# astro-turing/Integrating-diagenetic-equations-using-Python

Hardware: AMD Instinct MI355X
Metric: grid-point-steps/sec (5 fields, fp64) (higher is better)
Workload: dtype f64

## Files before the change

integrating-diagenetic-equations-using-python_amd/csrc/marl_kernels.h:

```cpp
#pragma once
#include <type_traits>

#include "marl_math.h"
#include "marl_brent.h"

namespace marl {

enum : int { LAYOUT_FIELD_MAJOR = 0, LAYOUT_TILED = 1 };

template <int LAYOUT>
__device__ __forceinline__ int64_t at(int f, int64_t i, int64_t ld)
{
    if constexpr (LAYOUT == LAYOUT_FIELD_MAJOR)
        return (int64_t)f * ld + i;
    else
        return (i >> 6) * (int64_t)(NF * 64) + f * 64 + (i & 63);
}

struct Slab {
    int64_t n_buf;
    int64_t goff;
    int64_t ld;
    int64_t out_lo;
    int64_t out_hi;
};

__device__ __forceinline__ double nanmin(double a, double b) { return (a < b || a != a) ? a : b; }
__device__ __forceinline__ double nanmax(double a, double b) { return (a > b || a != a) ? a : b; }
template <bool FINITE = false>
__device__ __forceinline__ double mon_min(double a, double b) { return FINITE ? __builtin_fmin(a, b) : nanmin(a, b); }
template <bool FINITE = false>
__device__ __forceinline__ double mon_max(double a, double b) { return FINITE ? __builtin_fmax(a, b) : nanmax(a, b); }


#ifdef MARL_LAB_PHASE_CLOCK
__device__ unsigned long long marl_lab_phase[8];
#define MARL_PHASE_MARK(k) do { const unsigned long long t_ = __builtin_amdgcn_s_memtime(); ph_acc[k] += t_ - ph_last; ph_last = t_; } while (0)
#else
#define MARL_PHASE_MARK(k) do { } while (0)
#endif

#define MARL_ONCE _Pragma("unroll") for (int once_ = 0; once_ < 1; once_++)
#define MARL_FIELDS _Pragma("unroll") for (int f = 0; f < NF; f++)

template <int BLK, bool REUSE = true, bool VD = false, int SEAM = 0>
struct StencilBlock {
    static constexpr int EDGE_DOUBLES = 2 * NF * BLK;
    static constexpr bool CACHE_LDS = PC_LDS_SLOTS > 0;
    static constexpr bool CACHE = REUSE && (EDGE_DOUBLES + TABLE_DOUBLES + PC_LDS_SLOTS * BLK) * 8 <= 60 * 1024;
    static constexpr int CACHE_DOUBLES = CACHE ? PC_LDS_SLOTS * BLK : 0;
    static constexpr int LDS_DOUBLES = EDGE_DOUBLES + TABLE_DOUBLES + CACHE_DOUBLES;

    double* lds;
    Tables T;
    HotConsts K;
    const DevConsts* C;
    int tid;
    int parity;
    unsigned masks;
    static constexpr bool EDGE_ONCE = CACHE;
    unsigned edge_cells;
    __device__ __forceinline__ bool edge_wave() const
    {
        if constexpr (EDGE_ONCE) return edge_cells & 1u;
        else return __builtin_amdgcn_ballot_w64(is_edge() != 0) != 0;
    }
    __device__ __forceinline__ unsigned is_first() const { return masks & 1u; }
    __device__ __forceinline__ unsigned is_last() const { return (masks >> 8) & 1u; }
    __device__ __forceinline__ unsigned in_zone() const { return (masks >> 16) & 1u; }
    __device__ __forceinline__ unsigned is_edge() const { return masks & 0x101u; }
    PointCache<(CACHE && CACHE_LDS) ? BLK : 0> cache;
    bool reuse_live = false;
    static constexpr int SEAM_STRIDE = 16, SEAM_READS = 0x10000, SEAM_WAVE0 = 0x20000, SEAM_WAVEW = 0x40000;
    static_assert(SEAM < BLK, "the recording lane is a lane of the window");
    double* seam = nullptr;
    int seam_pos = 0;
#ifdef MARL_LAB_PHASE_CLOCK
    unsigned long long ph_acc[6] = {0, 0, 0, 0, 0, 0}, ph_last = __builtin_amdgcn_s_memtime();
    __device__ __forceinline__ void phase_flush()
    {
        if (threadIdx.x == 0)
            for (int k = 0; k < 6; k++) atomicAdd(&marl_lab_phase[k], ph_acc[k]);
    }
#endif

    __device__ __forceinline__ StencilBlock(double* lds_, int64_t g0, const DevConsts* __restrict__ c)
        : lds(lds_), T(load_tables(lds_ + EDGE_DOUBLES, BLK)), K(load_hot(c)), C(c), tid(threadIdx.x), parity(0)
    {
        set_window(g0);
        if constexpr (CACHE && CACHE_LDS) cache.s = lds_ + EDGE_DOUBLES + TABLE_DOUBLES + tid;
    }

    __device__ __forceinline__ void rebind(int t)
    {
        tid = t;
        if constexpr (CACHE && CACHE_LDS) cache.s = lds + EDGE_DOUBLES + TABLE_DOUBLES + t;
    }

    __device__ __forceinline__ void set_window(int64_t g)
    {
        const int64_t N = C->N, mlo = C->mask_lo, mhi = C->mask_hi;
        masks = ((g == 0) ? 1u : 0u) | ((g == N - 1) ? 0x100u : 0u) | ((g >= mlo && g < mhi) ? 0x10000u : 0u);
        edge_cells = 0;
        if constexpr (EDGE_ONCE) edge_cells = (__builtin_amdgcn_ballot_w64(is_edge() != 0) != 0) ? 1u : 0u;
    }

    template <int MODE = TR_PLAIN>
    __device__ __forceinline__ void eval(const double (&ys)[NF], double (&k)[NF], PointAux& aux)
    {
        MARL_PHASE_MARK(4);
        double* e = lds + parity * (NF * BLK);
#pragma unroll
        for (int f = 0; f < NF; f++) e[f * BLK + tid] = ys[f];
        if constexpr (SEAM > 0) {
            if (seam_pos & SEAM_WAVEW) {
                int tw = tid;
                asm volatile("" : "+v"(tw));
                if (tw == SEAM) {
                    double* rec = seam + (seam_pos & 0xffff);
#pragma unroll
                    for (int f = 0; f < NF; f++) rec[f] = ys[f];
                }
            }
        }
        MARL_PHASE_MARK(0);
        PointLocal pl;
        MARL_ONCE point_local<CACHE ? MODE : TR_PLAIN, (CACHE && CACHE_LDS) ? BLK : 0, VD>(ys, in_zone(), K, C, T, pl, aux, cache, reuse_live);
        MARL_PHASE_MARK(1);
        __syncthreads();
        MARL_PHASE_MARK(2);
        const int tl = tid > 0 ? tid - 1 : 0;
        const int tr = tid < BLK - 1 ? tid + 1 : BLK - 1;
        double left[NF], right[NF];
#pragma unroll
        for (int f = 0; f < NF; f++) left[f] = e[f * BLK + tl];
        if constexpr (SEAM > 0) {
            if ((seam_pos & (SEAM_WAVE0 | SEAM_READS)) == (SEAM_WAVE0 | SEAM_READS)) {
                int t0 = tid;
                asm volatile("" : "+v"(t0));
                if (t0 == 0) {
                    const double* prev = seam + ((seam_pos & 0xffff) ^ 8);
#pragma unroll
                    for (int f = 0; f < NF; f++) left[f] = prev[f];
                }
            }
            seam_pos += SEAM_STRIDE;
        }
        const bool need_right_solids = __builtin_amdgcn_ballot_w64(!pl.upw) != 0;
        if constexpr (CACHE) {
#pragma unroll
            for (int f = 2; f < NF; f++) right[f] = e[f * BLK + tr];
            asm volatile("" : "=v"(right[0]), "=v"(right[1]));
            if (need_right_solids) {
                right[0] = e[tr];
                right[1] = e[BLK + tr];
            }
        } else {
#pragma unroll
            for (int f = 0; f < NF; f++) right[f] = (f >= 2 || need_right_solids) ? e[f * BLK + tr] : 0.0;
        }
        parity ^= 1;
        MARL_ONCE {
            double um[NF], up[NF];
#pragma unroll
            for (int f = 0; f < NF; f++) { um[f] = left[f]; up[f] = right[f]; }
            if (edge_wave()) {
                if (is_last()) {
#pragma unroll
                    for (int f = 0; f < NF; f++) up[f] = ghost_upper(f, ys[f], um[f]);
                }
                if (is_first()) {
#pragma unroll
                    for (int f = 0; f < NF; f++) um[f] = ghost_lower(C->bc[f], ys[f]);
                }
            }
            point_rates<VD, true, !CACHE>(ys, um, up, K, T, pl, k, need_right_solids);
        }
#ifdef MARL_LAB_PHASE_CLOCK
        asm volatile("" :: "v"(k[0]), "v"(k[4]));
        MARL_PHASE_MARK(3);
        ph_acc[5]++;
#endif
    }
};

template <int BLK, int NQ, int NMIN, bool FINITE = false>
__device__ __forceinline__ void block_reduce(double (&q)[NQ], double* scratch)
{
    const int lane = threadIdx.x & 63, wave = threadIdx.x >> 6;
    constexpr int NW = BLK / 64;
    auto combine = [](int j, double a, double o) { return (j == 0) ? a + o : (j <= NMIN ? mon_min<FINITE>(a, o) : mon_max<FINITE>(a, o)); };
    if constexpr (NW > 1) {
        __syncthreads();
#pragma unroll
        for (int j = 0; j < NQ; j++) scratch[j * BLK + threadIdx.x] = q[j];
        __syncthreads();
#pragma unroll
        for (int jj = 0; jj < (NQ + NW - 1) / NW; jj++) {
            const int j = wave + jj * NW;
            if (j < NQ) {
                double a = scratch[j * BLK + lane];
#pragma unroll
                for (int i = 1; i < NW; i++) a = combine(j, a, scratch[j * BLK + lane + 64 * i]);
#pragma unroll
                for (int off = 32; off > 0; off >>= 1) a = combine(j, a, __shfl_xor(a, off, 64));
                if (lane == 0) scratch[j * BLK] = a;
            }
        }
        __syncthreads();
        if (threadIdx.x == 0) {
#pragma unroll
            for (int j = 0; j < NQ; j++) q[j] = scratch[j * BLK];
        }
        __syncthreads();
    } else {
#pragma unroll
        for (int off = 32; off > 0; off >>= 1) {
#pragma unroll
            for (int j = 0; j < NQ; j++) q[j] = combine(j, q[j], __shfl_xor(q[j], off, 64));
        }
    }
}

struct ZBatch {
    int64_t zstride;
    const int32_t* act;
    int64_t act_stride;
    int want;
    const int32_t* list;
};
__device__ __forceinline__ int64_t z_inst(const ZBatch& B)
{
    return B.list ? (int64_t)__builtin_amdgcn_readfirstlane(B.list[blockIdx.z]) : (int64_t)blockIdx.z;
}
__device__ __forceinline__ bool z_masked_out(const ZBatch& B)
{
    return B.act && !(*reinterpret_cast<const int32_t*>(reinterpret_cast<const char*>(B.act) + z_inst(B) * B.act_stride) & B.want);
}
template <class P>
__device__ __forceinline__ P* z_shift(P* p, const ZBatch& B)
{
    return reinterpret_cast<P*>(reinterpret_cast<char*>(const_cast<typename std::remove_const<P>::type*>(p)) + z_inst(B) * B.zstride);
}

template <int LAYOUT, bool VD = false>
__global__ void __launch_bounds__(256) rhs_kernel(const double* __restrict__ y, double* __restrict__ dydt,
                                                  const DevConsts* __restrict__ consts, Slab S, int64_t inst_stride, int const_stride,
                                                  ZBatch B = ZBatch{0, nullptr, 0, 0, nullptr})
{
    if (z_masked_out(B)) return;
    __shared__ double tabs[TABLE_DOUBLES];
    const Tables T = load_tables(tabs, 256);
    const DevConsts& C = consts[blockIdx.y * const_stride + z_inst(B)];
    y = z_shift(y, B) + blockIdx.y * inst_stride;
    dydt = z_shift(dydt, B) + blockIdx.y * inst_stride;
    const int64_t l = (int64_t)blockIdx.x * 256 + threadIdx.x;
    if (l < S.out_lo || l >= S.out_hi) return;
    const int64_t g = l + S.goff;
    double uc[NF], um[NF], up[NF], r[NF];
    PointAux aux;
#pragma unroll
    for (int f = 0; f < NF; f++) {
        uc[f] = y[at<LAYOUT>(f, l, S.ld)];
        um[f] = (g > 0) ? y[at<LAYOUT>(f, l - 1, S.ld)] : ghost_lower(C.bc[f], uc[f]);
    }
#pragma unroll
    for (int f = 0; f < NF; f++) up[f] = (g < C.N - 1) ? y[at<LAYOUT>(f, l + 1, S.ld)] : ghost_upper(f, uc[f], um[f]);
    const HotConsts K = load_hot(&C);
    PointCache<0> pc;
    bool live = false;
    rhs_point<TR_PLAIN, 0, VD>(uc, um, up, g >= C.mask_lo && g < C.mask_hi, K, &C, T, r, aux, pc, live);
#pragma unroll
    for (int f = 0; f < NF; f++) dydt[at<LAYOUT>(f, l, S.ld)] = r[f];
}

__global__ void __launch_bounds__(256) math_probe_kernel(int op, const double* __restrict__ x, double* __restrict__ y, int64_t n, double e)
{
    __shared__ double tabs[TABLE_DOUBLES];
    const Tables T = load_tables(tabs, 256);
    const int64_t i = (int64_t)blockIdx.x * 256 + threadIdx.x;
    if (i >= n) return;
    const double v = x[i];
    double r;
    switch (op) {
        case 0: r = fast_log(v, T); break;
        case 1: r = fast_exp(v, T); break;
        case 2: r = pow_sat(v, e, T); break;
        case 3: r = rcp_nr(v); break;
        case 4: r = fv_sigma<false>(v, e, T); break;
        default: r = fv_sigma<true>(v, e, T); break;
    }
    y[i] = r;
}

template <int SRC, int DST>
__global__ void __launch_bounds__(256) convert_kernel(const double* __restrict__ src, double* __restrict__ dst, int64_t n,
                                                      int64_t ld_src, int64_t ld_dst, int64_t stride_src, int64_t stride_dst)
{
    src += blockIdx.y * stride_src;
    dst += blockIdx.y * stride_dst;
    const int64_t i = (int64_t)blockIdx.x * 256 + threadIdx.x;
    if (i >= n) return;
#pragma unroll
    for (int f = 0; f < NF; f++) dst[at<DST>(f, i, ld_dst)] = src[at<SRC>(f, i, ld_src)];
}

constexpr int NQ = 8;
constexpr int NQMIN = 4;

__device__ __forceinline__ void monitors_init(double (&q)[NQ])
{
    q[0] = 0.0;
    q[1] = q[2] = q[3] = q[4] = __builtin_inf();
    q[5] = q[6] = q[7] = -__builtin_inf();
}

template <bool FINITE = false>
__device__ __forceinline__ void monitors_accumulate(double (&q)[NQ], const double (&u)[NF], double U, double W)
{
    q[1] = mon_min<FINITE>(mon_min<FINITE>(mon_min<FINITE>(mon_min<FINITE>(mon_min<FINITE>(q[1], u[0]), u[1]), u[2]), u[3]), u[4]);
    q[2] = mon_min<FINITE>(q[2], u[0]);
    q[3] = mon_min<FINITE>(q[3], u[1]);
    q[4] = mon_min<FINITE>(q[4], U);
    q[5] = mon_max<FINITE>(q[5], u[0] + u[1]);
    q[6] = mon_max<FINITE>(q[6], u[4]);
    q[7] = mon_max<FINITE>(q[7], W);
}

template <int LAYOUT>
__global__ void __launch_bounds__(256) monitors_kernel(const double* __restrict__ y, const DevConsts* __restrict__ consts,
                                                       Slab S, int64_t inst_stride, double* __restrict__ part)
{
    __shared__ double scratch[NQ * 256];
    __shared__ double tabs[TABLE_DOUBLES];
    const Tables T = load_tables(tabs, 256);
    const DevConsts& C = consts[blockIdx.y];
    y += blockIdx.y * inst_stride;
    double q[NQ];
    monitors_init(q);
    for (int64_t l = S.out_lo + (int64_t)blockIdx.x * 256 + threadIdx.x; l < S.out_hi; l += (int64_t)gridDim.x * 256) {
        double u[NF];
#pragma unroll
        for (int f = 0; f < NF; f++) u[f] = y[at<LAYOUT>(f, l, S.ld)];
        const double Phi = u[4];
        const double F = 1.0 - fast_exp(10.0 - 10.0 * rcp_nr(Phi), T);
        const double rF = C.hot.rhorat * F;
        monitors_accumulate(q, u, C.hot.presum + rF * (Phi * Phi * Phi) * rcp_nr(1.0 - Phi), C.hot.presum - rF * Phi * Phi);
    }
    block_reduce<256, NQ, NQMIN>(q, scratch);
    if (threadIdx.x == 0) {
        double* p = part + ((int64_t)blockIdx.y * gridDim.x + blockIdx.x) * NQ;
#pragma unroll
        for (int j = 0; j < NQ; j++) p[j] = q[j];
    }
}

__global__ void __launch_bounds__(256) reduce_records_kernel(const double* __restrict__ part, int64_t nblocks, double* __restrict__ out)
{
    __shared__ double scratch[NQ * 256];
    part += (int64_t)blockIdx.x * nblocks * NQ;
    double q[NQ];
    monitors_init(q);
    for (int64_t b = threadIdx.x; b < nblocks; b += 256) {
#pragma unroll
        for (int j = 0; j < NQ; j++) {
            const double o = part[b * NQ + j];
            q[j] = (j == 0) ? q[j] + o : (j <= NQMIN ? nanmin(q[j], o) : nanmax(q[j], o));
        }
    }
    block_reduce<256, NQ, NQMIN>(q, scratch);
    if (threadIdx.x == 0) {
#pragma unroll
        for (int j = 0; j < NQ; j++) out[(int64_t)blockIdx.x * NQ + j] = q[j];
    }
}

__global__ void __launch_bounds__(256) reduce_chunks_kernel(const double* __restrict__ part, int64_t nrec, int64_t chunk, double* __restrict__ out)
{
    __shared__ double scratch[NQ * 256];
    const int64_t lo = (int64_t)blockIdx.x * chunk, hi = (lo + chunk < nrec) ? lo + chunk : nrec;
    double q[NQ];
    monitors_init(q);
    for (int64_t b = lo + threadIdx.x; b < hi; b += 256) {
#pragma unroll
        for (int j = 0; j < NQ; j++) {
            const double o = part[b * NQ + j];
            q[j] = (j == 0) ? q[j] + o : (j <= NQMIN ? nanmin(q[j], o) : nanmax(q[j], o));
        }
    }
    block_reduce<256, NQ, NQMIN>(q, scratch);
    if (threadIdx.x == 0) {
#pragma unroll
        for (int j = 0; j < NQ; j++) out[(int64_t)blockIdx.x * NQ + j] = q[j];
    }
}

template <int LAYOUT>
__device__ __forceinline__ void load_cells(const double* __restrict__ y, int64_t l, const Slab& S, const DevConsts& C, double (&u)[NF])
{
    const bool in = l >= 0 && l < S.n_buf;
#pragma unroll
    for (int f = 0; f < NF; f++) u[f] = in ? y[at<LAYOUT>(f, l, S.ld)] : C.bc[f];
}

#ifdef MARL_LAB_CLOCK
__device__ unsigned long long marl_lab_clock[3 * 16384];
#endif
template <int NSTEPS, class SB>
__device__ __forceinline__ void rk4_advance(SB& sb, double (&y)[NF], double dt)
{
    double ys[NF], k[NF], acc[NF];
    PointAux aux;
    const double h2 = 0.5 * dt, h6 = dt / 6.0;
#pragma unroll 1
    for (int step = 0; step < NSTEPS; step++) {
        sb.template eval<TR_AUTO>(y, k, aux);
        MARL_FIELDS { acc[f] = k[f]; ys[f] = y[f] + h2 * k[f]; }
        sb.template eval<TR_REUSE>(ys, k, aux);
        MARL_FIELDS { acc[f] = acc[f] + 2.0 * k[f]; ys[f] = y[f] + h2 * k[f]; }
        sb.template eval<TR_REUSE>(ys, k, aux);
        MARL_FIELDS { acc[f] = acc[f] + 2.0 * k[f]; ys[f] = y[f] + dt * k[f]; }
        sb.template eval<TR_REUSE>(ys, k, aux);
        MARL_FIELDS y[f] = y[f] + h6 * (acc[f] + k[f]);
    }
}

#ifndef MARL_LAB_RK4_WAVES_MIN
#define MARL_LAB_RK4_WAVES_MIN 4
#define MARL_LAB_RK4_WAVES_MAX 8
#endif
template <int BLK, int LAYOUT, int NSTEPS, bool VD = false>
__global__ void __launch_bounds__(BLK) __attribute__((amdgpu_waves_per_eu(MARL_LAB_RK4_WAVES_MIN, MARL_LAB_RK4_WAVES_MAX))) rk4_fused_kernel(const double* __restrict__ yin, double* __restrict__ yout,
                                                        const DevConsts* __restrict__ consts, Slab S, double dt)
{
#ifdef MARL_LAB_CLOCK
    const unsigned long long lab_t0 = __builtin_amdgcn_s_memtime(), lab_r0 = __builtin_amdgcn_s_memrealtime();
#endif
    constexpr int H = 4 * NSTEPS;
    constexpr int V = BLK - 2 * H;
    static_assert(V > 0, "window too small for the fused halo");
    using SB = StencilBlock<BLK, true, VD>;
    __shared__ double lds[SB::LDS_DOUBLES];
    const DevConsts& C = consts[0];

    const int64_t w0 = S.out_lo + (int64_t)blockIdx.x * V - H;
    const int64_t l = w0 + (int64_t)threadIdx.x;
    double y[NF];
    load_cells<LAYOUT>(yin, l, S, C, y);
    SB sb(lds, l + S.goff, consts);
    rk4_advance<NSTEPS>(sb, y, dt);

    const int wi = threadIdx.x;
    MARL_ONCE if (wi >= H && wi < BLK - H && l >= S.out_lo && l < S.out_hi) {
#pragma unroll
        for (int f = 0; f < NF; f++) yout[at<LAYOUT>(f, l, S.ld)] = y[f];
    }
#ifdef MARL_LAB_PHASE_CLOCK
    sb.phase_flush();
#endif
#ifdef MARL_LAB_CLOCK
    if (threadIdx.x == 0 && blockIdx.x < 16384) {
        marl_lab_clock[3 * blockIdx.x] = __builtin_amdgcn_s_memtime() - lab_t0;
        marl_lab_clock[3 * blockIdx.x + 1] = __builtin_amdgcn_s_memrealtime() - lab_r0;
        marl_lab_clock[3 * blockIdx.x + 2] = lab_r0;
    }
#endif
}

constexpr unsigned STREAM_SPIN_LIMIT = 1u << 19;

template <int BLK, int LAYOUT, int NSTEPS, bool VD = false>
__global__ void __launch_bounds__(BLK) __attribute__((amdgpu_waves_per_eu(4, 8)))
rk4_stream_kernel(double* bufA, double* bufB, const DevConsts* __restrict__ consts, Slab S, double dt, unsigned levels, unsigned tiles,
                  unsigned* queue, unsigned* done, unsigned* sticky, unsigned item_base, unsigned level_base, double* bufC = nullptr)
{
    constexpr int H = 4 * NSTEPS;
    constexpr int V = BLK - 2 * H;
    using SB = StencilBlock<BLK, true, VD>;
    __shared__ double lds[SB::LDS_DOUBLES];
    __shared__ unsigned s_item, s_abort;
    const DevConsts& C = consts[0];
    SB sb(lds, 0, consts);
    const unsigned total = levels * tiles;

#ifdef MARL_LAB_BROKEN_STREAM_LATCH
    if (threadIdx.x == 0) {
        s_item = __hip_atomic_fetch_add(&queue[0], 1u, __ATOMIC_RELAXED, __HIP_MEMORY_SCOPE_AGENT) - item_base;
        s_abort = 0;
    }
    while (true) {
        __syncthreads();
#else
    while (true) {
        __syncthreads();
        if (threadIdx.x == 0) {
            s_item = __hip_atomic_fetch_add(&queue[0], 1u, __ATOMIC_RELAXED, __HIP_MEMORY_SCOPE_AGENT) - item_base;
            s_abort = 0;
        }
        __syncthreads();
#endif
        const unsigned item = s_item;
        if (item >= total) break;
        const unsigned level = item / tiles, tile = item - level * tiles;
        if (level > 0) {
            if (threadIdx.x < 3) {
                const int64_t t = (int64_t)tile - 1 + threadIdx.x;
                if (t >= 0 && t < (int64_t)tiles) {
                    unsigned spins = 0;
                    while ((int)(__hip_atomic_load(&done[t], __ATOMIC_RELAXED, __HIP_MEMORY_SCOPE_AGENT) - (level_base + level)) < 0) {
                        __builtin_amdgcn_s_sleep(4);
                        if (++spins > STREAM_SPIN_LIMIT ||
                            ((spins & 255u) == 0 && __hip_atomic_load(sticky, __ATOMIC_RELAXED, __HIP_MEMORY_SCOPE_AGENT))) {
                            __hip_atomic_store(sticky, 1u, __ATOMIC_RELAXED, __HIP_MEMORY_SCOPE_AGENT);
                            s_abort = 1;
                            break;
                        }
                    }
                }
            }
            __syncthreads();
            if (s_abort) break;
        }
        const double* src = bufC ? (level == 0 ? bufA : ((level & 1u) ? bufB : bufC)) : ((level & 1u) ? bufB : bufA);
        double* dst = bufC ? (level + 1 == levels ? bufA : ((level & 1u) ? bufC : bufB)) : ((level & 1u) ? bufA : bufB);
        const int64_t l = S.out_lo + (int64_t)tile * V - H + threadIdx.x;
        const bool in = l >= 0 && l < S.n_buf;
        double y[NF];
#pragma unroll
        for (int f = 0; f < NF; f++)
            y[f] = in ? __hip_atomic_load(src + at<LAYOUT>(f, l, S.ld), __ATOMIC_RELAXED, __HIP_MEMORY_SCOPE_AGENT) : C.bc[f];
        sb.set_window(l + S.goff);
        sb.reuse_live = false;
        rk4_advance<NSTEPS>(sb, y, dt);
        if ((int)threadIdx.x >= H && (int)threadIdx.x < BLK - H && l >= S.out_lo && l < S.out_hi) {
#pragma unroll
            for (int f = 0; f < NF; f++) __hip_atomic_store(dst + at<LAYOUT>(f, l, S.ld), y[f], __ATOMIC_RELAXED, __HIP_MEMORY_SCOPE_AGENT);
        }
        __atomic_signal_fence(__ATOMIC_SEQ_CST);
        __builtin_amdgcn_s_waitcnt(0);
        __atomic_signal_fence(__ATOMIC_SEQ_CST);
        __syncthreads();
        if (threadIdx.x == 0) {
            __hip_atomic_store(&done[tile], level_base + level + 1u, __ATOMIC_RELAXED, __HIP_MEMORY_SCOPE_AGENT);
#ifdef MARL_LAB_BROKEN_STREAM_LATCH
            s_item = __hip_atomic_fetch_add(&queue[0], 1u, __ATOMIC_RELAXED, __HIP_MEMORY_SCOPE_AGENT) - item_base;
            s_abort = 0;
#endif
        }
    }
}

template <int BLK, int LAYOUT, int NSTEPS>
__global__ void __launch_bounds__(BLK) __attribute__((amdgpu_waves_per_eu(4, 8)))
rk4_chain_kernel(double* bufA, double* bufB, const DevConsts* __restrict__ consts, Slab S, double dt, unsigned levels, unsigned items,
                 unsigned* queue, unsigned* done, unsigned* sticky, unsigned item_base, unsigned level_base, double* bufC,
                 unsigned K, unsigned nsub_last, int64_t bound)
{
    constexpr int H = 4 * NSTEPS;
    constexpr int V = BLK - 2 * H;
    constexpr int W = BLK - H;
    static_assert(V > 0, "window too small for the fused halo");
    using SB = StencilBlock<BLK, true, false, BLK - H - 1>;
    __shared__ double lds[SB::LDS_DOUBLES];
    __shared__ double seam[H * SB::SEAM_STRIDE];
    __shared__ unsigned s_item, s_abort;
    const DevConsts& C = consts[0];
    SB sb(lds, 0, consts);
    sb.seam = seam;
    const unsigned total = levels * items;
    const unsigned chains = items - 1;

    while (true) {
        __syncthreads();
        if (threadIdx.x == 0) {
            s_item = __hip_atomic_fetch_add(&queue[0], 1u, __ATOMIC_RELAXED, __HIP_MEMORY_SCOPE_AGENT) - item_base;
            s_abort = 0;
        }
        __syncthreads();
        const unsigned item = __builtin_amdgcn_readfirstlane(s_item);
        if (item >= total) break;
        const unsigned level = item / items, tile = item - level * items;
        if (level > 0) {
            if (threadIdx.x < 3) {
                const int64_t t = (int64_t)tile - 1 + threadIdx.x;
                if (t >= 0 && t < (int64_t)items) {
                    unsigned spins = 0;
                    while ((int)(__hip_atomic_load(&done[t], __ATOMIC_RELAXED, __HIP_MEMORY_SCOPE_AGENT) - (level_base + level)) < 0) {
                        __builtin_amdgcn_s_sleep(4);
                        if (++spins > STREAM_SPIN_LIMIT ||
                            ((spins & 255u) == 0 && __hip_atomic_load(sticky, __ATOMIC_RELAXED, __HIP_MEMORY_SCOPE_AGENT))) {
                            __hip_atomic_store(sticky, 1u, __ATOMIC_RELAXED, __HIP_MEMORY_SCOPE_AGENT);
                            s_abort = 1;
                            break;
                        }
                    }
                }
            }
            __syncthreads();
            if (s_abort) break;
        }
        const double* src = bufC ? (level == 0 ? bufA : ((level & 1u) ? bufB : bufC)) : ((level & 1u) ? bufB : bufA);
        double* dst = bufC ? (level + 1 == levels ? bufA : ((level & 1u) ? bufC : bufB)) : ((level & 1u) ? bufA : bufB);
        const bool chain = tile < chains;
        const unsigned nsub = chain ? (tile + 1 == chains ? nsub_last : K) : 1u;
        const int64_t first = S.out_lo - H + (chain ? (int64_t)tile * (V + (int64_t)W * (K - 1)) : bound);
        const int64_t clip = chain ? S.out_lo + bound : S.out_hi;
#pragma unroll 1
        for (unsigned j = 0; j < nsub; j++) {
            int tid = threadIdx.x;
            asm volatile("" : "+v"(tid));
            sb.rebind(tid);
            const int64_t l = first + (int64_t)j * W + tid;
            const bool in = l >= 0 && l < S.n_buf;
            double y[NF];
#pragma unroll
            for (int f = 0; f < NF; f++)
                y[f] = in ? __hip_atomic_load(src + at<LAYOUT>(f, l, S.ld), __ATOMIC_RELAXED, __HIP_MEMORY_SCOPE_AGENT) : C.bc[f];
            sb.set_window(l + S.goff);
            sb.reuse_live = false;
            sb.seam_pos = __builtin_amdgcn_readfirstlane((int)(j & 1u) * 8 + (j ? SB::SEAM_READS : 0) + (tid < 64 ? SB::SEAM_WAVE0 : 0)
                                                         + (tid / 64 == (BLK - H - 1) / 64 ? SB::SEAM_WAVEW : 0));
            rk4_advance<NSTEPS>(sb, y, dt);
            const int lo = j ? 0 : H;
            int ts = threadIdx.x;
            asm volatile("" : "+v"(ts));
            const int64_t ls = first + (int64_t)j * W + ts;
            if (ts >= lo && ts < BLK - H && ls < clip) {
#pragma unroll
                for (int f = 0; f < NF; f++) __hip_atomic_store(dst + at<LAYOUT>(f, ls, S.ld), y[f], __ATOMIC_RELAXED, __HIP_MEMORY_SCOPE_AGENT);
            }
        }
        __atomic_signal_fence(__ATOMIC_SEQ_CST);
        __builtin_amdgcn_s_waitcnt(0);
        __atomic_signal_fence(__ATOMIC_SEQ_CST);
        __syncthreads();
        if (threadIdx.x == 0) __hip_atomic_store(&done[tile], level_base + level + 1u, __ATOMIC_RELAXED, __HIP_MEMORY_SCOPE_AGENT);
    }
}

namespace dp {
constexpr double A21 = 1.0 / 5;
constexpr double A31 = 3.0 / 40, A32 = 9.0 / 40;
constexpr double A41 = 44.0 / 45, A42 = -56.0 / 15, A43 = 32.0 / 9;
constexpr double A51 = 19372.0 / 6561, A52 = -25360.0 / 2187, A53 = 64448.0 / 6561, A54 = -212.0 / 729;
constexpr double A61 = 9017.0 / 3168, A62 = -355.0 / 33, A63 = 46732.0 / 5247, A64 = 49.0 / 176, A65 = -5103.0 / 18656;
constexpr double B1 = 35.0 / 384, B3 = 500.0 / 1113, B4 = 125.0 / 192, B5 = -2187.0 / 6784, B6 = 11.0 / 84;
constexpr double E1 = -71.0 / 57600, E3 = 71.0 / 16695, E4 = -71.0 / 1920, E5 = 17253.0 / 339200, E6 = -22.0 / 525, E7 = 1.0 / 40;
constexpr double SAFETY = 0.9, MIN_FACTOR = 0.2, MAX_FACTOR = 10.0;
constexpr double P[7][4] = {
    {1, -8048581381.0 / 2820520608, 8663915743.0 / 2820520608, -12715105075.0 / 11282082432},
    {0, 0, 0, 0},
    {0, 131558114200.0 / 32700410799, -68118460800.0 / 10900136933, 87487479700.0 / 32700410799},
    {0, -1754552775.0 / 470086768, 14199869525.0 / 1410260304, -10690763975.0 / 1880347072},
    {0, 127303824393.0 / 49829197408, -318862633887.0 / 49829197408, 701980252875.0 / 199316789632},
    {0, -282668133.0 / 205662961, 2019193451.0 / 616988883, -1453857185.0 / 822651844},
    {0, 40617522.0 / 29380423, -110615467.0 / 29380423, 69997945.0 / 29380423}};
}


enum : int { ST_DONE = 0, ST_RUNNING = 1, ST_BUDGET = 2, ST_PAUSED = 3, ST_TOO_SMALL = -1 };

struct Rk45Ctrl {
    double t, h_abs, t_bound, rtol, atol;
    double h_try, t_new;
    double t_old, h_prev;
    double err_norm;
    double pause_t;
    double g[7];
    double ev_first[7];
    double ev_last[7];
    int64_t n_events[7];
    int64_t nfev, n_acc, n_rej, attempts, max_attempts;
    int64_t n_total;
    int32_t status;
    int32_t cur;
    int32_t rejected;
    int32_t accepted_last;
    int32_t pause_on_event;
    int32_t event_fired;
};

__device__ __forceinline__ void rk45_prepare_attempt(Rk45Ctrl& c)
{
    const double min_step = 10.0 * fabs(nextafter(c.t, __builtin_inf()) - c.t);
    if (!c.rejected) {
        if (c.h_abs < min_step) c.h_abs = min_step;
    } else if (c.h_abs < min_step) {
        c.status = ST_TOO_SMALL;
        return;
    }
    if (c.max_attempts > 0 && c.attempts >= c.max_attempts) {
        c.status = ST_BUDGET;
        return;
    }
    double t_new = c.t + c.h_abs;
    if (t_new - c.t_bound > 0.0) t_new = c.t_bound;
    c.t_new = t_new;
    c.h_try = t_new - c.t;
    c.h_abs = fabs(c.h_try);
    c.attempts++;
}

__device__ __forceinline__ bool rk45_decide(Rk45Ctrl& c, double sumsq, const Tables* T = nullptr)
{
    const double err = sqrt(sumsq) / sqrt((double)c.n_total);
    c.err_norm = err;
    c.nfev += 6;
    double f;
    if (T && err > 1e-300 && err < 1e300) f = dp::SAFETY * fast_exp(-0.2 * fast_log(err, *T), *T);
    else f = dp::SAFETY * pow(err, -0.2);
    if (err < 1.0) {
        double factor = (err == 0.0) ? dp::MAX_FACTOR : ((f < dp::MAX_FACTOR) ? f : dp::MAX_FACTOR);
        if (c.rejected && !(factor < 1.0)) factor = 1.0;
        c.h_abs *= factor;
        c.accepted_last = 1;
        c.rejected = 0;
        c.n_acc++;
        c.t_old = c.t;
        c.h_prev = c.h_try;
        c.t = c.t_new;
        c.cur ^= 1;
        return true;
    }
    c.h_abs *= (f > dp::MIN_FACTOR) ? f : dp::MIN_FACTOR;
    c.accepted_last = 0;
    c.rejected = 1;
    c.n_rej++;
    return false;
}

__device__ __forceinline__ bool rk45_decide_lean(Rk45Ctrl& c, double sumsq, double inv_n, const Tables& T)
{
    const double e2 = sumsq * inv_n;
    c.err_norm = e2;
    c.nfev += 6;
    double f;
    if (e2 > 1e-300 && e2 < 1e300) f = dp::SAFETY * fast_exp(-0.1 * fast_log(e2, T), T);
    else f = dp::SAFETY * pow(sqrt(e2), -0.2);
    if (e2 < 1.0) {
        double factor = (e2 == 0.0) ? dp::MAX_FACTOR : ((f < dp::MAX_FACTOR) ? f : dp::MAX_FACTOR);
        if (c.rejected && !(factor < 1.0)) factor = 1.0;
        c.h_abs *= factor;
        c.accepted_last = 1;
        c.rejected = 0;
        c.n_acc++;
        c.t_old = c.t;
        c.h_prev = c.h_try;
        c.t = c.t_new;
        c.cur ^= 1;
        return true;
    }
    c.h_abs *= (f > dp::MIN_FACTOR) ? f : dp::MIN_FACTOR;
    c.accepted_last = 0;
    c.rejected = 1;
    c.n_rej++;
    return false;
}

__device__ __forceinline__ void rk45_prepare_attempt_lean(Rk45Ctrl& c)
{
    if (!(c.h_abs > fabs(c.t) * 0x1p-48) || c.t == 0.0) {
        rk45_prepare_attempt(c);
        return;
    }
    if (c.max_attempts > 0 && c.attempts >= c.max_attempts) {
        c.status = ST_BUDGET;
        return;
    }
    double t_new = c.t + c.h_abs;
    if (t_new - c.t_bound > 0.0) t_new = c.t_bound;
    c.t_new = t_new;
    c.h_try = t_new - c.t;
    c.h_abs = fabs(c.h_try);
    c.attempts++;
}

__device__ __forceinline__ int rk45_event_one(Rk45Ctrl& c, int e, double gn)
{
    const double go = c.g[e];
    int fired = 0;
    const bool up = go <= 0.0 && gn >= 0.0, down = go >= 0.0 && gn <= 0.0;
    if (up || down) {
        const double d = go - gn;
        const double tc = (d != 0.0) ? c.t_old + c.h_prev * (go / d) : c.t;
        if (c.n_events[e] == 0) c.ev_first[e] = tc;
        c.ev_last[e] = tc;
        c.n_events[e]++;
        fired = 1;
    }
    c.g[e] = gn;
    return fired;
}

__device__ __forceinline__ double rk45_monitor_of_record(const double* rec, int e)
{
    const int slot = (e < 3) ? e + 1 : (e == 3 ? 5 : (e == 4 ? 6 : (e == 5 ? 4 : 7)));
    return (e == 3 || e == 4) ? rec[slot] - 1.0 : rec[slot];
}

__device__ __forceinline__ int rk45_monitor_slot(int e)
{
    return (e < 3) ? e + 1 : (e == 3 ? 5 : (e == 4 ? 6 : (e == 5 ? 4 : 7)));
}

__device__ __forceinline__ int rk45_events(Rk45Ctrl& c, const double (&rec)[NQ])
{
    int fired = 0;
#pragma unroll
    for (int e = 0; e < 7; e++) fired |= rk45_event_one(c, e, rk45_monitor_of_record(rec, e));
    return fired;
}

__device__ __forceinline__ void rk45_advance_status(Rk45Ctrl& c, bool accepted, int fired)
{
    if (accepted) {
        if (c.t - c.t_bound >= 0.0) {
            c.status = ST_DONE;
        } else if (c.t >= c.pause_t || (fired && c.pause_on_event)) {
            c.status = ST_PAUSED;
            c.event_fired = fired;
        }
    }
    if (c.status == ST_RUNNING) rk45_prepare_attempt(c);
}

__device__ __forceinline__ void rk45_advance_status_no_events(Rk45Ctrl& c)
{
    if (c.t - c.t_bound >= 0.0) c.status = ST_DONE;
    else if (c.t >= c.pause_t) c.status = ST_PAUSED;
    if (c.status == ST_RUNNING) rk45_prepare_attempt(c);
}

__device__ __forceinline__ void rk45_finish_attempt(Rk45Ctrl& c, const double (&rec)[NQ], const Tables* T = nullptr)
{
    const bool accepted = rk45_decide(c, rec[0], T);
    const int fired = accepted ? rk45_events(c, rec) : 0;
    rk45_advance_status(c, accepted, fired);
}

__global__ void rk45_init_kernel(Rk45Ctrl* ctrl, const double* __restrict__ rec0, double t0, double t1, double first_step,
                                 double rtol, double atol, int64_t n_total, int64_t max_attempts, int32_t cur)
{
    Rk45Ctrl c = {};
    c.t = t0; c.t_bound = t1; c.h_abs = first_step; c.rtol = rtol; c.atol = atol;
    c.t_old = t0; c.pause_t = __builtin_inf();
    c.n_total = n_total; c.max_attempts = max_attempts; c.cur = cur;
    c.nfev = 1;
    c.status = (t0 == t1) ? ST_DONE : ST_RUNNING;
    const double* r = rec0 + (int64_t)blockIdx.x * NQ;
    const double g0[7] = {r[1], r[2], r[3], r[5] - 1.0, r[6] - 1.0, r[4], r[7]};
    for (int e = 0; e < 7; e++) c.g[e] = g0[e];
    if (c.status == ST_RUNNING) rk45_prepare_attempt(c);
    ctrl[blockIdx.x] = c;
}

__global__ void rk45_resume_kernel(Rk45Ctrl* ctrl, double pause_t, int64_t max_attempts)
{
    Rk45Ctrl& c = ctrl[blockIdx.x];
    c.pause_t = pause_t;
    c.max_attempts = max_attempts;
    if (c.status == ST_PAUSED || c.status == ST_BUDGET) {
        c.status = ST_RUNNING;
        c.event_fired = 0;
        rk45_prepare_attempt(c);
    }
}

constexpr int CONTROL_THREADS = 512;
__global__ void __launch_bounds__(CONTROL_THREADS) rk45_control_kernel(const double* __restrict__ recs, int64_t nrec, Rk45Ctrl* ctrl)
{
    __shared__ double scratch[NQ * CONTROL_THREADS];
#ifdef MARL_CTL_CLOCK
    const unsigned long long c0 = __builtin_amdgcn_s_memrealtime();
#endif
    const int32_t status = ctrl->status;
    double q[NQ];
    monitors_init(q);
    for (int64_t b = threadIdx.x; b < nrec; b += CONTROL_THREADS) {
        double o[NQ];
#pragma unroll
        for (int j = 0; j < NQ; j++) o[j] = recs[b * NQ + j];
#pragma unroll
        for (int j = 0; j < NQ; j++) q[j] = (j == 0) ? q[j] + o[j] : (j <= NQMIN ? nanmin(q[j], o[j]) : nanmax(q[j], o[j]));
    }
    if (status != ST_RUNNING) return;
#ifdef MARL_CTL_CLOCK
    const unsigned long long c1 = __builtin_amdgcn_s_memrealtime();
#endif
    block_reduce<CONTROL_THREADS, NQ, NQMIN>(q, scratch);
#ifdef MARL_CTL_CLOCK
    const unsigned long long c2 = __builtin_amdgcn_s_memrealtime();
#endif
    if (threadIdx.x == 0) {
        Rk45Ctrl c = *ctrl;
        rk45_finish_attempt(c, q);
        *ctrl = c;
#ifdef MARL_CTL_CLOCK
        const unsigned long long c3 = __builtin_amdgcn_s_memrealtime();
        if (c.attempts == 300) printf("CTLCLOCK load %llu reduce %llu finish %llu (x10 ns)\n", c1 - c0, c2 - c1, c3 - c2);
#endif
    }
}

struct DenseWeights { double w[7]; };

template <int BLK, bool DENSE = false, class SB = StencilBlock<BLK>, int PARK = 0, bool EITHER = false>
__device__ __forceinline__ void dp45_attempt(SB& sb, double h, const double (&y)[NF], const double (&k1)[NF],
                                             double (&yn)[NF], double (&k7)[NF], double (&esum)[NF],
                                             PointAux& aux, const DenseWeights& dw = DenseWeights{}, const double* pk = nullptr,
                                             bool dense_now = false)
{
    static_assert(!(EITHER && DENSE), "EITHER chooses at run time");
#define MARL_SEPARATE_BLOCKS() MARL_FIELDS asm volatile("" : "+v"(esum[f]))
    const double e1 = DENSE ? dw.w[0] : dp::E1, e3 = DENSE ? dw.w[2] : dp::E3, e4 = DENSE ? dw.w[3] : dp::E4;
    const double e5 = DENSE ? dw.w[4] : dp::E5, e6 = DENSE ? dw.w[5] : dp::E6, e7 = DENSE ? dw.w[6] : dp::E7;
    double ys[NF], k2[NF], k3[NF], k4[NF], kk[NF], s6[NF], bn[NF];
#define MARL_Y(f) ((f) < PARK ? pk[(f) * BLK] : y[f])
    MARL_FIELDS ys[f] = MARL_Y(f) + (k1[f] * dp::A21) * h;
    sb.template eval<TR_FILL>(ys, k2, aux);
    MARL_FIELDS ys[f] = MARL_Y(f) + (k1[f] * dp::A31 + k2[f] * dp::A32) * h;
    sb.template eval<TR_REUSE>(ys, k3, aux);
    MARL_FIELDS ys[f] = MARL_Y(f) + (k1[f] * dp::A41 + k2[f] * dp::A42 + k3[f] * dp::A43) * h;
    sb.template eval<TR_REUSE>(ys, k4, aux);
    MARL_FIELDS {
        ys[f] = MARL_Y(f) + (k1[f] * dp::A51 + k2[f] * dp::A52 + k3[f] * dp::A53 + k4[f] * dp::A54) * h;
        s6[f] = k1[f] * dp::A61 + k2[f] * dp::A62 + k3[f] * dp::A63 + k4[f] * dp::A64;
        bn[f] = k1[f] * dp::B1 + k3[f] * dp::B3 + k4[f] * dp::B4;
        if constexpr (!EITHER) esum[f] = k1[f] * e1 + k3[f] * e3 + k4[f] * e4;
    }
    if constexpr (EITHER) {
        if (dense_now) {
            MARL_FIELDS esum[f] = k1[f] * dw.w[0] + k3[f] * dw.w[2] + k4[f] * dw.w[3];
// ... 1059 lines not shown
```

Before: 51.53 billion.

## Add wave-uniform interior fast path and reload kernel args from kernarg segment

```diff
diff --git a/integrating-diagenetic-equations-using-python_amd/csrc/marl_kernels.h b/integrating-diagenetic-equations-using-python_amd/csrc/marl_kernels.h
--- a/integrating-diagenetic-equations-using-python_amd/csrc/marl_kernels.h
+++ b/integrating-diagenetic-equations-using-python_amd/csrc/marl_kernels.h
@@ -62,12 +62,18 @@
     unsigned edge_cells;
     __device__ __forceinline__ bool edge_wave() const
     {
-        if constexpr (EDGE_ONCE) return edge_cells & 1u;
+        if constexpr (SEAM > 0) {
+            unsigned e = edge_cells;
+            asm volatile("" : "+s"(e));
+            return e & 1u;
+        } else if constexpr (EDGE_ONCE) return edge_cells & 1u;
         else return __builtin_amdgcn_ballot_w64(is_edge() != 0) != 0;
     }
-    __device__ __forceinline__ unsigned is_first() const { return masks & 1u; }
-    __device__ __forceinline__ unsigned is_last() const { return (masks >> 8) & 1u; }
-    __device__ __forceinline__ unsigned in_zone() const { return (masks >> 16) & 1u; }
+    bool w_zone = false;
+    __device__ __forceinline__ unsigned edge_word() const { unsigned e = edge_cells; asm volatile("" : "+s"(e)); return e; }
+    __device__ __forceinline__ unsigned is_first() const { if constexpr (SEAM > 0) return (unsigned)tid + 1u == ((edge_word() >> 8) & 0x1ffu); else return masks & 1u; }
+    __device__ __forceinline__ unsigned is_last() const { if constexpr (SEAM > 0) return (unsigned)tid + 1u == ((edge_word() >> 20) & 0x1ffu); else return (masks >> 8) & 1u; }
+    __device__ __forceinline__ unsigned in_zone() const { if constexpr (SEAM > 0) return w_zone; else return (masks >> 16) & 1u; }
     __device__ __forceinline__ unsigned is_edge() const { return masks & 0x101u; }
     PointCache<(CACHE && CACHE_LDS) ? BLK : 0> cache;
     bool reuse_live = false;
@@ -87,7 +93,8 @@
     __device__ __forceinline__ StencilBlock(double* lds_, int64_t g0, const DevConsts* __restrict__ c)
         : lds(lds_), T(load_tables(lds_ + EDGE_DOUBLES, BLK)), K(load_hot(c)), C(c), tid(threadIdx.x), parity(0)
     {
-        set_window(g0);
+        if constexpr (SEAM > 0) set_interior(false);
+        else set_window(g0);
         if constexpr (CACHE && CACHE_LDS) cache.s = lds_ + EDGE_DOUBLES + TABLE_DOUBLES + tid;
     }
 
@@ -103,6 +110,27 @@
         masks = ((g == 0) ? 1u : 0u) | ((g == N - 1) ? 0x100u : 0u) | ((g >= mlo && g < mhi) ? 0x10000u : 0u);
         edge_cells = 0;
         if constexpr (EDGE_ONCE) edge_cells = (__builtin_amdgcn_ballot_w64(is_edge() != 0) != 0) ? 1u : 0u;
+    }
+
+    __device__ __forceinline__ void set_window_seam(int64_t gw)
+    {
+        const int64_t N = C->N, mlo = C->mask_lo, mhi = C->mask_hi;
+        const int64_t g = gw + tid;
+        w_zone = g >= mlo && g < mhi;
+        masks = 0;
+        const int wave = __builtin_amdgcn_readfirstlane(tid) >> 6;
+        const int64_t t0 = -gw, t1 = N - 1 - gw;
+        unsigned e = 0;
+        if (t0 >= 0 && t0 < BLK) e |= (((unsigned)t0 + 1u) << 8) | ((int)(t0 >> 6) == wave ? 1u : 0u);
+        if (t1 >= 0 && t1 < BLK) e |= (((unsigned)t1 + 1u) << 20) | ((int)(t1 >> 6) == wave ? 1u : 0u);
+        edge_cells = __builtin_amdgcn_readfirstlane(e);
+    }
+
+    __device__ __forceinline__ void set_interior(bool zone)
+    {
+        w_zone = zone;
+        masks = 0;
+        edge_cells = 0;
     }
 
     template <int MODE = TR_PLAIN>
@@ -169,7 +197,18 @@
 #pragma unroll
                     for (int f = 0; f < NF; f++) up[f] = ghost_upper(f, ys[f], um[f]);
                 }
-                if (is_first()) {
+                if constexpr (SEAM > 0) {
+                    size_t off = offsetof(DevConsts, bc);
+                    asm volatile("" : "+s"(off));
+                    const double* bcp = reinterpret_cast<const double*>(reinterpret_cast<const char*>(C) + off);
+                    double bcv[NF];
+#pragma unroll
+                    for (int f = 0; f < NF; f++) bcv[f] = bcp[f];
+                    if (is_first()) {
+#pragma unroll
+                        for (int f = 0; f < NF; f++) um[f] = ghost_lower(bcv[f], ys[f]);
+                    }
+                } else if (is_first()) {
 #pragma unroll
                     for (int f = 0; f < NF; f++) um[f] = ghost_lower(C->bc[f], ys[f]);
                 }
@@ -550,6 +589,28 @@
     }
 }
 
+struct ChainArgs {
+    double *bufA, *bufB;
+    const DevConsts* consts;
+    Slab S;
+    double dt;
+    unsigned levels, items;
+    unsigned *queue, *done, *sticky;
+    unsigned item_base, level_base;
+    double* bufC;
+    unsigned K, nsub_last;
+    int64_t bound;
+};
+static_assert(offsetof(ChainArgs, S) == 24 && offsetof(ChainArgs, dt) == 64 && offsetof(ChainArgs, queue) == 80 && offsetof(ChainArgs, bufC) == 112 &&
+              offsetof(ChainArgs, bound) == 128 && sizeof(ChainArgs) == 136, "the argument list of rk4_chain_kernel, in order");
+typedef const __attribute__((address_space(4))) ChainArgs* ChainArgsPtr;
+__device__ __forceinline__ ChainArgsPtr chain_args()
+{
+    ChainArgsPtr a = (ChainArgsPtr)__builtin_amdgcn_kernarg_segment_ptr();
+    asm volatile("" : "+s"(a));
+    return a;
+}
+
 template <int BLK, int LAYOUT, int NSTEPS>
 __global__ void __launch_bounds__(BLK) __attribute__((amdgpu_waves_per_eu(4, 8)))
 rk4_chain_kernel(double* bufA, double* bufB, const DevConsts* __restrict__ consts, Slab S, double dt, unsigned levels, unsigned items,
@@ -567,11 +628,17 @@
     const DevConsts& C = consts[0];
     SB sb(lds, 0, consts);
     sb.seam = seam;
+    dt = pin_uniform(dt);
     const unsigned total = levels * items;
     const unsigned chains = items - 1;
 
     while (true) {
         __syncthreads();
+        typedef __attribute__((address_space(1))) unsigned* GlobalWords;
+        ChainArgsPtr G = chain_args();
+        unsigned *const queue = (unsigned*)(GlobalWords)G->queue, *const done = (unsigned*)(GlobalWords)G->done,
+                 *const sticky = (unsigned*)(GlobalWords)G->sticky;
+        const unsigned items = G->items, item_base = G->item_base, level_base = G->level_base;
         if (threadIdx.x == 0) {
             s_item = __hip_atomic_fetch_add(&queue[0], 1u, __ATOMIC_RELAXED, __HIP_MEMORY_SCOPE_AGENT) - item_base;
             s_abort = 0;
@@ -599,35 +666,78 @@
             __syncthreads();
             if (s_abort) break;
         }
-        const double* src = bufC ? (level == 0 ? bufA : ((level & 1u) ? bufB : bufC)) : ((level & 1u) ? bufB : bufA);
-        double* dst = bufC ? (level + 1 == levels ? bufA : ((level & 1u) ? bufC : bufB)) : ((level & 1u) ? bufA : bufB);
-        const bool chain = tile < chains;
-        const unsigned nsub = chain ? (tile + 1 == chains ? nsub_last : K) : 1u;
-        const int64_t first = S.out_lo - H + (chain ? (int64_t)tile * (V + (int64_t)W * (K - 1)) : bound);
-        const int64_t clip = chain ? S.out_lo + bound : S.out_hi;
+        const double* src;
+        double* dst;
+        unsigned nsub;
+        int64_t first, clip;
+        {
+            ChainArgsPtr A = chain_args();
+            double *const pA = A->bufA, *const pB = A->bufB, *const pC = A->bufC;
+            const unsigned nlev = A->levels, KK = A->K, nlast = A->nsub_last;
+            const int64_t olo = A->S.out_lo, ohi = A->S.out_hi, bnd = A->bound;
+            src = (const double*)(const __attribute__((address_space(1))) double*)(pC ? (level == 0 ? pA : ((level & 1u) ? pB : pC)) : ((level & 1u) ? pB : pA));
+            dst = (double*)(__attribute__((address_space(1))) double*)(pC ? (level + 1 == nlev ? pA : ((level & 1u) ? pC : pB)) : ((level & 1u) ? pA : pB));
+            const bool chain = tile < chains;
+            nsub = chain ? (tile + 1 == chains ? nlast : KK) : 1u;
+            first = olo - H + (chain ? (int64_t)tile * (V + (int64_t)W * (KK - 1)) : bnd);
+            clip = chain ? olo + bnd : ohi;
+        }
 #pragma unroll 1
         for (unsigned j = 0; j < nsub; j++) {
             int tid = threadIdx.x;
             asm volatile("" : "+v"(tid));
             sb.rebind(tid);
-            const int64_t l = first + (int64_t)j * W + tid;
-            const bool in = l >= 0 && l < S.n_buf;
+            ChainArgsPtr A = chain_args();
+            const int64_t n_buf = A->S.n_buf, goff = A->S.goff, ld = A->S.ld;
+            const int64_t lw = first + (int64_t)j * W, gw = lw + goff;
+            const int64_t mlo = C.mask_lo, mhi = C.mask_hi;
+            auto neg = [](int64_t a, int64_t b) {
+                int32_t hi = (int32_t)(((uint64_t)a - (uint64_t)b) >> 32);
+                asm("" : "+s"(hi));
+                return hi;
+            };
+            const int32_t out_any = neg(lw, 0) | neg(n_buf, lw + BLK) | neg(gw, 1) | neg(C.N - 1, gw + BLK);
+            const int32_t zone_part = neg(gw, mlo) | neg(mhi, gw + BLK);
+            const int32_t zone_some = neg(mlo, gw + BLK) & neg(gw, mhi);
+            const bool interior = out_any >= 0 && (zone_part >= 0 || zone_some >= 0);
+            const int64_t l = lw + tid;
+            bool in = true;
+            int64_t la = l;
+            if (!interior) {
+                asm volatile("");
+                in = l >= 0 && l < n_buf;
+                la = in ? l : 0;
+            }
             double y[NF];
 #pragma unroll
-            for (int f = 0; f < NF; f++)
-                y[f] = in ? __hip_atomic_load(src + at<LAYOUT>(f, l, S.ld), __ATOMIC_RELAXED, __HIP_MEMORY_SCOPE_AGENT) : C.bc[f];
-            sb.set_window(l + S.goff);
+            for (int f = 0; f < NF; f++) y[f] = __hip_atomic_load(src + at<LAYOUT>(f, la, ld), __ATOMIC_RELAXED, __HIP_MEMORY_SCOPE_AGENT);
+            if (interior) {
+                sb.set_interior(zone_part >= 0);
+            } else {
+                asm volatile("");
+#pragma unroll
+                for (int f = 0; f < NF; f++) y[f] = in ? y[f] : C.bc[f];
+                sb.set_window_seam(gw);
+            }
             sb.reuse_live = false;
-            sb.seam_pos = __builtin_amdgcn_readfirstlane((int)(j & 1u) * 8 + (j ? SB::SEAM_READS : 0) + (tid < 64 ? SB::SEAM_WAVE0 : 0)
-                                                         + (tid / 64 == (BLK - H - 1) / 64 ? SB::SEAM_WAVEW : 0));
+            const int wave = __builtin_amdgcn_readfirstlane(tid) >> 6;
+            sb.seam_pos = (int)(j & 1u) * 8 + (j ? SB::SEAM_READS : 0) + (wave == 0 ? SB::SEAM_WAVE0 : 0)
+                          + (wave == (BLK - H - 1) / 64 ? SB::SEAM_WAVEW : 0);
+            const int64_t room = clip - lw;
+            int hi = neg(room, BLK - H) < 0 ? (int)room : BLK - H;
+            asm volatile("" : "+s"(hi));
             rk4_advance<NSTEPS>(sb, y, dt);
-            const int lo = j ? 0 : H;
+            int sp = sb.seam_pos;
+            asm volatile("" : "+s"(sp));
+            const int lo = (sp & SB::SEAM_READS) ? 0 : H;
             int ts = threadIdx.x;
             asm volatile("" : "+v"(ts));
             const int64_t ls = first + (int64_t)j * W + ts;
-            if (ts >= lo && ts < BLK - H && ls < clip) {
-#pragma unroll
-                for (int f = 0; f < NF; f++) __hip_atomic_store(dst + at<LAYOUT>(f, ls, S.ld), y[f], __ATOMIC_RELAXED, __HIP_MEMORY_SCOPE_AGENT);
+            if (ts >= lo && ts < hi) {
+                int64_t lds_ = 0;
+                if constexpr (LAYOUT == LAYOUT_FIELD_MAJOR) lds_ = chain_args()->S.ld;
+#pragma unroll
+                for (int f = 0; f < NF; f++) __hip_atomic_store(dst + at<LAYOUT>(f, ls, lds_), y[f], __ATOMIC_RELAXED, __HIP_MEMORY_SCOPE_AGENT);
             }
         }
         __atomic_signal_fence(__ATOMIC_SEQ_CST);
```

Measured after the change: 52.20 billion, median of 6. +1.3%, better.
